# Pi-Star-Lab/RESCO

Hardware: AMD Instinct MI355X
Metric: env-steps/sec (higher is better)
Workload: dtype f32; 1 GPU; ingolstadt21 x 4096 lock-step envs per GPU (BASELINE config 3), fixed demand from the map's rou.xml, on-device seeded random policy, Krauss sigma 0.5 + speedFactor dev 0.1; tls_expiry=1, map=ingolstadt21, envs_per_gpu=4096, pipes=2, ticks_per_env_step=10, block_threads=512, lds_bytes_per_env=40896, parallelism=env-batch split x1, no collective on the data path

## Files before the change

### resco_amd/csrc/resco_step.h

```cpp
#pragma once
#include "resco_tables.h"

struct State {
    char *base;
    size_t nc;
    int32_t *trip_log;
    int32_t *env;
    int32_t *tls;
    long long *stats;
    uint16_t *dep_next;
    uint32_t *mail;
    RS_HD float *pos() const { return (float *)base; }
    RS_HD float *speed() const { return RS_G((float *)(base + 4 * nc)); }
    RS_HD float *accel() const { return RS_G((float *)(base + 8 * nc)); }
    RS_HD float *tloss() const { return RS_G((float *)(base + 12 * nc)); }
    RS_HD float *sf() const { return RS_G((float *)(base + 16 * nc)); }
    RS_HD uint32_t *coop(int par) const { return RS_G((uint32_t *)(base + (par ? 43 : 20) * nc)); }
    RS_HD uint32_t *cooplead(int par) const { return RS_G((uint32_t *)(base + (par ? 47 : 24) * nc)); }
    RS_HD uint16_t *lane() const { return RS_G((uint16_t *)(base + 28 * nc)); }
    RS_HD uint16_t *trip() const { return RS_G((uint16_t *)(base + 30 * nc)); }
    RS_HD uint16_t *cursor() const { return RS_G((uint16_t *)(base + 32 * nc)); }
    RS_HD uint16_t *swait() const { return RS_G((uint16_t *)(base + 34 * nc)); }
    RS_HD uint16_t *rwait() const { return RS_G((uint16_t *)(base + 36 * nc)); }
    RS_HD uint16_t *depart() const { return RS_G((uint16_t *)(base + 38 * nc)); }
// ... 423 lines not shown
template <class LT> RS_DEV Found leader_found(const LT &L, const Grid &grid, int cell0, int ncell, float pos, int k, int self, float win) {
    const int c = cell_of(L, pos, ncell);
    const unsigned long long mykey = order_key(pos, k);
    Found f{(int)NIL, ~0ull, 0u, 0u};
    const uint32_t cw = grid.c[cell0 + c];
    int s = ((cw ^ grid.tag) & CELL_TAG) ? (int)NIL : (int)(cw & NIL);
    if (s == self && ((cw >> CELL_CNT_SHIFT) & CELL_CNT_MAX) == 1u) s = NIL;
    while (s != NIL) {
        RS_ASSERT(s != self || order_key(L.node[s].pos, L.node[s].trip) == mykey)
        RS_CHAIN_STEP(f, s, (key > mykey) & (key < f.key))
    }
    if (f.slot == NIL && c + 1 < ncell) {
        const int cc = scan_up(grid, cell0 + c + 1, cell0 + cell_of(L, pos + win, ncell));
        if (cc >= 0) f = chain_rearmost(L, cell_head(grid, cc));
    }
    if (f.slot != NIL && f.pos() - pos > win) f.slot = NIL;
    return f;
}
template <class LT> RS_DEV int leader_within(const LT &L, const Grid &grid, int cell0, int ncell, float pos, int k, int self, float win) {
    return leader_found(L, grid, cell0, ncell, pos, k, self, win).slot;
}
template <class LT> RS_DEV int follower_within(const LT &L, const Grid &grid, int cell0, int ncell, float pos, int k, int self, float win) {
    const int c = cell_of(L, pos, ncell);
    const unsigned long long mykey = order_key(pos, k);
    Found f{(int)NIL, 0ull, 0u, 0u};
    for (int s = cell_head(grid, cell0 + c); s != NIL;) {
        RS_ASSERT(s != self || order_key(L.node[s].pos, L.node[s].trip) == mykey)
        RS_CHAIN_STEP(f, s, (key < mykey) & (key > f.key))
    }
    if (f.slot == NIL && c > 0) {
        const float lo = pos - win;
        const int cc = scan_down(grid, cell0 + (lo > 0.0f ? cell_of(L, lo, ncell) : 0), cell0 + c - 1);
        if (cc >= 0) f = chain_frontmost(L, cell_head(grid, cc));
    }
    if (f.slot != NIL && pos - f.pos() > win) f.slot = NIL;
    (void)self;
    return f.slot;
}
template <class LT> RS_DEV int at_or_behind_within(const LT &L, const Grid &grid, int cell0, int ncell, float back, float win) {
    if (back < 0.0f) return NIL;
    const int c = cell_of(L, back, ncell);
    Found f{(int)NIL, 0ull, 0u, 0u};
    for (int s = cell_head(grid, cell0 + c); s != NIL;) RS_CHAIN_STEP(f, s, !(nd_.pos > back) & (key > f.key))
    if (f.slot == NIL && c > 0) {
        const float lo = back - win;
        const int cc = scan_down(grid, cell0 + (lo > 0.0f ? cell_of(L, lo, ncell) : 0), cell0 + c - 1);
        if (cc >= 0) f = chain_frontmost(L, cell_head(grid, cc));
    }
    if (f.slot != NIL && back - f.pos() > win) f.slot = NIL;
    return f.slot;
}

template <class LT> RS_DEV int tls_state(const KTab &T, const LT &L, int tls, int pos) {
    if (tls == 0xFF) return TLS_G;
    return L.tstate[tls * T.tls_maxl + pos];
}
RS_DEV uint16_t cache_link(const KTab &T, const LaneRec &LR, int lane, int rq, int trip) {
    if (LR.link_cnt == 0) return NLINK_NONE;
    if (LR.flags & LF_INTERNAL) { const int l = LR.link_start; return (uint16_t)(l | (T.links()[l].arr_idx >= 0 ? NLINK_ARR : 0)); }
    return T.next_link()[((size_t)rq * T.kmax + (lane - (int)LR.edge_lane0)) * 2 + (trip & 1)];
}
template <class LT> RS_DEV bool foe_blocked(const KTab &T, const LT &L, const Grid &grid, const LinkRec &K) {
    for (int i = K.foe_start; i < K.foe_start + K.foe_cnt; ++i) {
        const FoeRec F = rec_load16(T.foes(), i);
        if (F.tls != 0xFF && tls_state(T, L, F.tls, F.tls_pos) == TLS_R) continue;
        if (F.arr_idx >= 0 && L.arr[F.arr_idx] < RM_FOE_GAP_Q) return true;
        if (F.via1_cell0 != 0xFFFF && cells_have_mover(grid, F.via1_cell0, F.via1_nc)) return true;
        if (F.via2_cell0 != 0xFFFF && cells_have_mover(grid, F.via2_cell0, F.via2_nc)) return true;
    }
    return false;
}
template <class LT> RS_DEV void tls_refresh(const KTab &T, const LT &L, const KParams &P, int s, int ph) {
    const int w = T.tls_maxl >> 2;
    const uint32_t *src = (const uint32_t *)((P.fixed_program ? T.cold.fix8 + T.cold.fix_state_off[s] : T.cold.tls8 + T.cold.tls_state_off[s]) + ph * T.tls_maxl);
    uint32_t *dst = (uint32_t *)((uint8_t *)L.tstate + s * T.tls_maxl);
    uint32_t v[8];
#pragma unroll
    for (int i = 0; i < 8; ++i) v[i] = src[i < w ? i : 0];
#pragma unroll
    for (int i = 0; i < 8; ++i) if (i < w) dst[i] = v[i];
#pragma unroll 1
    for (int i = 8; i < w; ++i) dst[i] = src[i];
}
template <class LT> RS_DEV void set_phase(const KTab &T, const LT &L, const KParams &P, int s, int ph) {
    if (ph < 0 || ph >= T.cold.tls_nphase[s]) return;
    L.phase[s] = ph;
    L.left[s] = P.tls_expiry ? T.cold.tls_dur[T.cold.tls_dur_off[s] + ph] : RM_TLS_HOLD_TICKS;
    tls_refresh(T, L, P, s, ph);
}
template <class LT> RS_DEV void tls_begin_of_tick(const KTab &T, const LT &L, const KParams &P, int s, int tick) {
    if (P.do_fsm && !P.fixed_program && tick == T.yellow_length) set_phase(T, L, P, s, L.nextp[s]);
    int left = L.left[s];
    if (left == 0) {
        const int32_t *dur = P.fixed_program ? T.cold.fix_dur + T.cold.fix_dur_off[s] : T.cold.tls_dur + T.cold.tls_dur_off[s];
        const int Pn = P.fixed_program ? T.cold.fix_nphase[s] : T.cold.tls_nphase[s];
        const int ph = (L.phase[s] + 1) % Pn;
        left = dur[ph];
        L.phase[s] = ph;
        tls_refresh(T, L, P, s, ph);
    }
    L.left[s] = left - 1;
}
struct ContRow { float c[4]; const float *cn; };
RS_DEV ContRow cont_row(const KTab &T, int rq) {
    ContRow R;
    R.cn = T.route_cont() + (size_t)rq * T.kmax;
    for (int j = 0; j < 4; ++j) R.c[j] = j < T.kmax ? R.cn[j] : 0.0f;
    return R;
}
RS_DEV float cont_of(const ContRow &R, int j) {
    return j == 0 ? R.c[0] : (j == 1 ? R.c[1] : (j == 2 ? R.c[2] : (j == 3 ? R.c[3] : R.cn[j])));
}
#define OCC_NONE (Grid{(uint16_t *)0, 0u})
#define OCC_FULL (Grid{(uint16_t *)1, 0u})
RS_DEV bool cont_notbest(float c) { return rs_float_as_int(c) < 0; }
RS_DEV float cont_len(float c) { return rs_int_as_float(rs_float_as_int(c) & 0x7FFFFFFF); }
RS_DEV int strategic_dir(const ContRow &R, int kk, int n, float x, float v, int extra, float &rem, const Grid &grid, int cell0, int nc, float occ_unit) {
    const float mine = cont_of(R, kk);
    rem = cont_len(mine) - x;
#ifdef RS_EMU_CHECK_MAIL
    { float best = 0.0f; for (int j = 0; j < n; ++j) { const float c = cont_len(cont_of(R, j)); if (c > best) best = c; }
      for (int j = 0; j < n; ++j) RS_ASSERT(cont_notbest(cont_of(R, j)) == !(cont_len(cont_of(R, j)) >= best - RM_CONT_EPS)) }
#endif
    if (!cont_notbest(mine)) return 0;
    int dl = 1000, dr = 1000;
    for (int j = kk + 1; j < n; ++j) if (!cont_notbest(cont_of(R, j))) { dl = j - kk; break; }
    for (int j = kk - 1; j >= 0; --j) if (!cont_notbest(cont_of(R, j))) { dr = kk - j; break; }
    const int dir = (dr <= dl) ? -1 : +1;
    if (grid.c == (uint16_t *)1) return dir;
    const int off = (dr <= dl ? dr : dl) + extra;
    const float la = (v > RM_LOOK_MIN_SPEED ? v : RM_LOOK_MIN_SPEED) * RM_LOOK_TIME + RM_LOOK_BASE;
    int cnt = 0;
    if (grid.c != (uint16_t *)0) cnt = cells_count(grid, cell0 + ((dr <= dl) ? -dr : dl) * nc, nc);
    if (rem - (float)cnt * occ_unit >= la * (float)off) return 0;
    return dir;
}
RS_DEV uint32_t link_reg_word(const KTab &T, int nlk) { return ((const uint32_t *)&T.links()[nlk & 0x7FFF])[2]; }
template <class LT> RS_DEV void register_approach_w(const KTab &T, const LT &L, uint32_t kw, float v, float pos, float lane_len, int vt) {
    const int st = tls_state(T, L, (int)((kw >> 16) & 0xFFu), (int)(kw >> 24));
    if (st == TLS_R) return;
    const float dist = lane_len - pos;
    if (st == TLS_Y && dist >= d_brake_gap(v, L.vtp[vt * VT_COLS + VT_DECEL])) return;
    const float ta = RS_DIV(dist, v > 1.0f ? v : 1.0f);
    const int q = ta * 10.0f >= 65000.0f ? 65000 : (int)(ta * 10.0f);
    rs_atomic_min(&L.arr[(int16_t)(kw & 0xFFFFu)], q);
}
template <class LT> RS_DEV void register_approach(const KTab &T, const LT &L, int nlk, float v, float pos, float lane_len, int vt) {
    if (!(nlk & NLINK_ARR)) return;
    if (v <= RM_HALT_SPEED) return;
    register_approach_w(T, L, link_reg_word(T, nlk), v, pos, lane_len, vt);
}
template <class LT> RS_DEV void follow_neighbour(const KTab &T, const LT &L, uint32_t key, bool clamp_gap, const LaneRec &LR, int lane, float x, float v,
                             float b, float tau, float mingap, float &vsafe) {
    const int X = (int)(key & 0xFFFFu), kx = (int)(key >> 16);
    if ((int)L.node[X].trip != kx) return;
    const int lx = L.aux[X].lane;
    if (lx == (int)LANE_NONE || (LR.flags & LF_INTERNAL)) return;
    const int l0 = LR.edge_lane0, n = LR.flags >> 2;
    if (lx < l0 || lx >= l0 + n) return;
    const float *vo = L.vtp + L.node[X].vt * VT_COLS;
    const float px = L.node[X].pos, backx = px - vo[VT_LENGTH];
    if (clamp_gap ? !(px >= x) : !(backx >= x)) return;
    float g = backx - x - mingap;
    if (clamp_gap && g < 0.0f) g = 0.0f;
    float vs = d_follow_speed(g, L.node[X].speed, b, vo[VT_DECEL], tau);
    float vc = v - b; if (vc < 0.0f) vc = 0.0f;
    if (vs < vc) vs = vc;
    if (vs < vsafe) vsafe = vs;
    (void)lane;
}

template <class LT> RS_DEV void mail_flag_set(const LT &L, int s, int par) { rs_atomic_or((uint32_t *)((Node *)L.node + s) + 3, SFQ_MAIL(par) << 16); }
template <class LT> RS_DEV void mail_flag_clear(const LT &L, int s, int par) { rs_atomic_and((uint32_t *)((Node *)L.node + s) + 3, ~(SFQ_MAIL(par) << 16)); }
template <class LT, class LP> RS_DEV void list_push(const LT &L, const LP &list, int counter, int s);
template <class LT> RS_DEV void flag_mover(const LT &L, int s, int t, int lct = 0) {
    uint32_t *w = (uint32_t *)((Node *)L.node + s) + 3;
    const uint32_t bit = (uint32_t)fl_mh(t) << 8;
    if (!(rs_atomic_fetch_or(w, bit | ((uint32_t)lct << 8)) & bit)) list_push(L, L.ls_mh, SC_NMH + (t & 1), s);
}
template <class LT, class LP> RS_DEV void list_push(const LT &L, const LP &list, int counter, int s) {
    const int i = rs_wave_ticket(&L.sc[counter]);
    if (i < (int)L.lcap) list[i] = (uint16_t)s;
}
RS_DEV float plan_vfree(const float *vt, float v, float lane_vmax, float sf) {
// ... 348 lines not shown
            }
            if (safe) {
                if (dir == dir_allowed) code = dir > 0 ? LCT_LEFT : LCT_RIGHT;
            } else if (want == 2) {
                if (lead_t != NIL) { G.cooplead(t & 1)[eo + s] = ((uint32_t)L.node[lead_t].trip << 16) | (uint32_t)lead_t; mail_flag_set(L, s, t & 1); }
                const int R = at_or_behind_within(L, grid, tcell0, nc, x - vt[VT_LENGTH], RM_COOP_RANGE);
                if (R != NIL) { rs_atomic_min(&G.coop(t & 1)[eo + R], ((uint32_t)k << 16) | (uint32_t)s); mail_flag_set(L, R, t & 1); }
            }
        }
    }
    if (sdir != 0 && (t % RM_SWAP_EVERY) == 0 && v <= RM_HALT_SPEED && rem <= RM_URGENT_DIST &&
        my_wait >= RM_SWAP_WAIT) {
        const int b = overlapping(L, grid, (int)LR.cell0 + sdir * nc, nc, x, k, s, vt[VT_LENGTH]);
        if (b != NIL) {
            const Node nb = L.node[b];
            float rem_b;
            if (nb.speed <= RM_HALT_SPEED && (int)L.aux[b].swait >= RM_SWAP_WAIT &&
                strategic_dir(cont_row(T, L.aux[b].rq), kk + sdir, n, nb.pos, nb.speed, 0, rem_b, grid, (int)LR.cell0 + sdir * nc, nc, T.occ_unit) == -sdir && rem_b <= RM_URGENT_DIST &&
                overlapping(L, grid, LR.cell0, nc, nb.pos, nb.trip, b, L.vtp[nb.vt * VT_COLS + VT_LENGTH]) == s)
                code |= sdir > 0 ? LCT_SWAP_LEFT : LCT_SWAP_RIGHT;
        }
    }
        return code;
}

template <class LT> RS_DEV bool phase_insert_decide(const KTab &T, const LT &L, const Grid &grid, int t, int d) {
    if ((int)L.dep_t[d] > t) return false;
    const int k = L.dep[d];
    const DepInfo LR = rec_load8(T.cold.dep_info, d);
    const float *vt = L.vtp + T.trip_vtype()[k] * VT_COLS;
    const float mypos = vt[VT_LENGTH] < LR.len ? vt[VT_LENGTH] : LR.len;
    const int nc = (int)(LR.len * L.cell_inv) + 1;
    const int c1 = LR.cell0 + cell_of(L, mypos + vt[VT_MINGAP] + T.maxlen, nc);
    for (int c = scan_up(grid, LR.cell0, c1); c >= 0; c = (c < c1 ? scan_up(grid, c + 1, c1) : -1))
        for (int o = cell_head(grid, c); o != NIL;) { RS_CHAIN_GUARD
            const Node od = L.node[o];
            const float back = (od.pos + L.vnx[o]) - L.vtp[od.vt * VT_COLS + VT_LENGTH];
            if (back - mypos - vt[VT_MINGAP] < 0.0f) return false;
            o = od.nxt;
        }
    return true;
}

template <class LT> RS_DEV int nth_free_slot(const LT &L, int C, int r) {
#pragma unroll 1
    for (int w = 0; w < (C + 31) / 32; ++w) {
        uint32_t fr = ~L.alive0[w];
        if (w == (C - 1) / 32 && (C & 31)) fr &= (1u << (C & 31)) - 1u;
        const int c = rs_popc(fr);
        if (r >= c) { r -= c; continue; }
#pragma unroll 1
        for (int j = 0; j < r; ++j) fr &= fr - 1u;
        return w * 32 + rs_ffs(fr) - 1;
    }
    return -1;
}

template <class LT> RS_DEV void lc_decide_and_flag(const KTab &T, const LT &L, const Grid &grid, const State &G, size_t eo, int t, int s) {
    const Aux ax = L.aux[s];
    if (ax.lane == LANE_NONE) return;
    const int code = phase_lc_decide(T, L, grid, G, eo, t, s, ax, L.node[s]);
    if (code) flag_mover(L, s, t, code);
}
struct ExecInline {};

template <int CAP, class Exec, class LT>
RS_DEV void rs_step_body_on(Exec &ex, const LT &L, const KTab &T, const State &G, const Out &O, const KParams &P,
                            const int32_t *actions, int env) {
    const int B = ex.B;
    const int C = CAP ? CAP : T.capacity, S = T.n_signals, NO = T.n_obs;
    const int genv = P.env_base + env;
    const size_t eo = (size_t)env * C;
    const int n_ticks = P.n_ticks;

    uint16_t *const grid0 = L.grid;

    ex.phase(0, [&](int tid) {
        if (tid < SC_STATS + ST_N) L.sc[tid] = tid < 4 ? G.env[env * 4 + tid] : 0;
        for (int i = tid; i < T.n_vtypes * VT_COLS; i += B) L.vtp[i] = T.cold.vtype_params[i];
        for (int i = tid; i < (int)(L.gstride >> 1); i += B) ((uint32_t *)grid0)[i] = 0x07FF07FFu;
        for (int i = tid; i < T.n_arr; i += B) L.arr[i] = ARR_NONE;
        for (int i = tid; i < (C + 31) / 32; i += B) { L.alive[i] = 0u; L.mailw[i] = 0u; }
        for (int i = tid; i < (T.n_dep + 31) / 32; i += B) L.insm[i] = 0u;
        for (int i = tid; i < T.n_dep; i += B) {
            const int k = G.dep_next[(size_t)env * T.n_dep + i];
            L.dep[i] = (uint16_t)k;
            L.dep_t[i] = k == (int)TRIP_NONE ? (uint16_t)0xFFFF : (uint16_t)T.cold.trip_depart[k];
        }
        for (int i = tid; i < S; i += B) {
            const int ph = G.tls[(env * S + i) * TLS_W + 0];
            L.phase[i] = ph;
            L.left[i] = G.tls[(env * S + i) * TLS_W + 1];
            L.nextp[i] = G.tls[(env * S + i) * TLS_W + 2];
            L.sig_arr[i] = 0; L.sig_dep[i] = G.tls[(env * S + i) * TLS_W + 3];
            tls_refresh(T, L, P, i, ph);
        }
    });
    ex.phase(1, [&](int tid) {
        const int hw0 = L.sc[SC_HW];
        for (int s = tid; s < C; s += B) {
            uint16_t ln = LANE_NONE, tr = TRIP_NONE;
            if (s < hw0) { ln = G.lane()[eo + s]; tr = G.trip()[eo + s]; }
            Aux ax; ax.lane = ln; ax.rq = 0; ax.nlink = NLINK_NONE; ax.swait = 0;
            if (ln == LANE_NONE) { L.aux[s] = ax; L.node[s].trip = TRIP_NONE; continue; }
            const float sp = G.speed()[eo + s], x = G.pos()[eo + s];
            const int rq = (int)T.routes()[T.trip_route()[tr]].start + (int)G.cursor()[eo + s];
            const LaneRec LR0 = rec_load16(T.lanes(), ln);
            ax.rq = (uint16_t)rq;
            ax.nlink = cache_link(T, LR0, ln, rq, tr);
            ax.swait = G.swait()[eo + s];
            L.aux[s] = ax;
            Node nn; nn.pos = x; nn.speed = sp; nn.trip = tr; nn.vt = T.trip_vtype()[tr];
            nn.fl = 0; nn.sfq = (uint16_t)speed_factor_q(P, genv, tr, L.vtp + nn.vt * VT_COLS);
            if ((G.mail[(size_t)env * ((C + 31) / 32) + (s >> 5)] >> (s & 31)) & 1u) nn.sfq |= (uint16_t)SFQ_MAIL((L.sc[SC_T] + 1) & 1);
            nn.nxt = grid_push(Grid{grid0, 0u}, LR0.cell0 + cell_of(L, x, lane_cells(L, LR0)), s, sp > RM_HALT_SPEED);
            if (n_ticks > 0) nn.fl = (uint8_t)classify(T, L, s, L.vtp + nn.vt * VT_COLS, sp, x, LR0, ln, rq, T.notbest()[rq], tr, sf_of(nn.sfq), L.sc[SC_T]);
            L.node[s] = nn;
            rs_atomic_or(&L.alive[s >> 5], 1u << (s & 31));
        }
        for (int s = B - 1 - tid; s < S; s += B) {
            if (P.do_fsm && !P.fixed_program) {
                const int a = actions[env * S + s], cur = L.phase[s], Gn = T.cold.tls_ngreen[s];
                if (a < 0 || a >= T.cold.tls_nphase[s]) L.nextp[s] = cur;
                else {
                    L.nextp[s] = a;
                    if (cur != a && cur < Gn && a < Gn) {
                        const int y = T.cold.tls_yellow[T.cold.tls_yel_off[s] + cur * Gn + a];
                        if (y >= 0) set_phase(T, L, P, s, y);
                    }
                }
            }
            if (n_ticks > 0) tls_begin_of_tick(T, L, P, s, 0);
        }
    });
    if (n_ticks > 0) ex.phase(2, [&](int tid) {
        const int hw = L.sc[SC_HW];
        for (int s = tid; s < hw; s += B) {
            const Aux ax = L.aux[s];
            if (ax.lane == LANE_NONE) continue;
            const Node me = L.node[s];
            register_approach(T, L, ax.nlink, me.speed, me.pos, T.lanes()[ax.lane].len, me.vt);
        }
    });

    int cur = 0;
    for (int tick = 0; tick < n_ticks; ++tick) {
        const int t = L.sc[SC_T], hw = L.sc[cur ? SC_HWNEW : SC_HW];
        const Grid gold{grid0, cur ? CELL_TAG : 0u}, gnew{grid0, cur ? 0u : CELL_TAG};
        const bool more = tick + 1 < n_ticks;
        const int lcap = (int)L.lcap;
        const int nwv = B >> 6;
        ex.phase(4, [&](int tid) {
            const int wv = ex.wave_of(tid), ln = tid & 63;
            const int nh = L.sc[SC_NH], nlc = L.sc[SC_NLC];
            const unsigned long long r0 = ex.role_begin();
            int role = 0;
            if (nh > lcap || nlc > lcap) {
                for (int pass = 0; pass < 2; ++pass)
                    for (int w = tid; w < hw; w += B) {
                        if (pass && !(L.node[w].fl & FL_LC)) continue;
                        if (pass) lc_decide_and_flag(T, L, gold, G, eo, t, w);
                        else phase_plan<true>(T, L, gold, G, eo, P, genv, t, w);
                    }
            } else {
                const int hch = (nh + RS_H_CHUNK - 1) / RS_H_CHUNK, lch = (nlc + RS_LIST_CHUNK - 1) / RS_LIST_CHUNK;
                const int total = hch + lch + ((hw + 63) >> 6);
                for (int it = 0;; ++it) {
                    const int c = ex.next_chunk(&L.sc[SC_CHUNK_P], wv, it, nwv);
                    if (c >= total) break;
                    if (c < hch) {
                        role = 1;
                        const int w = c * RS_H_CHUNK + ln;
                        if (ln < RS_H_CHUNK && w < nh) phase_plan<true>(T, L, gold, G, eo, P, genv, t, L.ls_h[w]);
                    } else if (c < hch + lch) {
                        role = 2;
                        const int w = (c - hch) * RS_LIST_CHUNK + ln;
                        if (ln < RS_LIST_CHUNK && w < nlc) lc_decide_and_flag(T, L, gold, G, eo, t, L.ls_lc[w]);
                    } else {
                        const int w = (c - hch - lch) * 64 + ln;
                        if (w < hw && !(L.node[w].fl & FL_H)) phase_plan<false>(T, L, gold, G, eo, P, genv, t, w);
                    }
                }
            }
            ex.role_end(role == 1 ? 7 : (role == 2 ? 8 : 9), r0);
            for (int i = tid; i < (T.n_dep + 31) / 32; i += B) L.insm[i] = 0u;
        });
        ex.phase(5, [&](int tid) {
            for (int i = tid; i < T.n_arr; i += B) L.arr[i] = ARR_NONE;
            for (int i = tid; i < (C + 31) / 32; i += B) L.alive0[i] = L.alive[i];
            int Bs = B;
            RS_OPAQUE_S(Bs)
            for (int i = tid; i < (int)(L.gstride >> 2); i += Bs) {
                unsigned long long *q = (unsigned long long *)grid0 + i;
                const unsigned long long w = *q;
                const unsigned long long st = ((w ^ grid_tag4(gold)) >> 15) & 0x0001000100010001ull;
                if (st) { const unsigned long long m = st * 0xFFFFull; *q = (w & ~m) | ((0x07FF07FF07FF07FFull | grid_tag4(gold)) & m); }
            }
            for (int d = B - 1 - tid; d < T.n_dep; d += B)
                if (phase_insert_decide(T, L, gold, t, d)) rs_atomic_or(&L.insm[d >> 5], 1u << (d & 31));
            if (more)
                for (int sg = B - 1 - tid; sg < S; sg += B) tls_begin_of_tick(T, L, P, sg, tick + 1);
            if (tid == 0) {
                L.sc[SC_T] = t + 1; L.sc[SC_STATS + ST_TICKS] += 1;
                L.sc[cur ? SC_HW : SC_HWNEW] = 0;
                L.sc[SC_ROOM] = C - L.sc[SC_NACT];
                L.sc[SC_NH] = 0; L.sc[SC_NLC] = 0;
                L.sc[SC_NMH + ((t + 1) & 1)] = 0;
                L.sc[SC_CHUNK_P] = 0; L.sc[SC_CHUNK_M] = 0;
            }
        });
        ex.phase(6, [&](int tid) {
            int active = 0, halted = 0, top = 0;
            const int wv = ex.wave_of(tid), ln = tid & 63;
            const int nmh = L.sc[SC_NMH + (t & 1)];
            int ich = 0;
// ... 35 lines not shown
                        L.aux[s] = na;
                        G.sf()[eo + s] = sfn; G.tloss()[eo + s] = 0.0f; G.cooplead(0)[eo + s] = COOP_NONE; G.cooplead(1)[eo + s] = COOP_NONE; G.coop(0)[eo + s] = COOP_NONE; G.coop(1)[eo + s] = COOP_NONE;
                        G.rwait()[eo + s] = 0; G.owner()[eo + s] = OWNER_NONE; G.depart()[eo + s] = (uint16_t)(t + 1); G.accel()[eo + s] = 0.0f; G.wtot()[eo + s] = 0;
                        {
                            const int k2 = T.cold.trip_next[k];
                            L.dep[d] = (uint16_t)k2;
                            L.dep_t[d] = k2 == (int)TRIP_NONE ? (uint16_t)0xFFFF : (uint16_t)T.cold.trip_depart[k2];
                        }
                        rs_atomic_or(&L.alive[s >> 5], 1u << (s & 31));
                        rs_atomic_add(&L.sc[SC_NACT], 1);
                        rs_atomic_add(&L.sc[SC_NINS], 1);
                        rs_atomic_add(&L.sc[SC_STATS + ST_INSERTED], 1);
                        rs_atomic_add(&L.sc[SC_STATS + ST_DEPDELAY], t - T.cold.trip_depart[k]);
                        if (s + 1 > top) top = s + 1;
                    }
                } else {
                    const int w = (c - mch - ich) * 64 + ln;
                    if (w < hw && (L.alive0[w >> 5] & (1u << (w & 31)))) {
                        if (all) phase_move<true>(T, L, gnew, G, P, env, eo, t, !more, more, w, active, halted, top);
                        else if (!(L.node[w].fl & fl_mh(t))) phase_move<false>(T, L, gnew, G, P, env, eo, t, !more, more, w, active, halted, top);
                    }
                }
            }
            ex.role_end(list ? 10 : 3, r0);
            rs_wave_add(&L.sc[SC_STATS + ST_ACTIVE_TICKS], active);
            rs_wave_add(&L.sc[SC_STATS + ST_WAITING], halted);
            rs_wave_max(&L.sc[cur ? SC_HW : SC_HWNEW], top);
            ex.role_end(15, r0);
        });
        cur ^= 1;
    }
    const int hw_end = L.sc[cur ? SC_HWNEW : SC_HW];

    const bool obs = P.do_observe != 0;
    if (obs) ex.phase(11, [&](int tid) {
        for (int i = tid; i < NO; i += B) { L.agg_q[i] = 0; L.agg_a[i] = 0; L.agg_w[i] = 0; L.agg_m[i] = 0; L.agg_s[i] = 0; L.agg_n[i] = 0; }
    });
    ex.phase(12, [&](int tid) {
        const int hw0 = G.env[env * 4 + 2];
        const int top = hw_end > hw0 ? hw_end : hw0;
        int hi = 0;
        for (int s = tid; s < top; s += B) {
            const int lane = L.aux[s].lane;
            G.lane()[eo + s] = (uint16_t)lane; G.trip()[eo + s] = L.node[s].trip;
            if (lane == (int)LANE_NONE) continue;
            hi = s + 1;
            if (L.node[s].sfq & SFQ_MAIL((L.sc[SC_T] + 1) & 1)) rs_atomic_or(&L.mailw[s >> 5], 1u << (s & 31));
            const int rq = L.aux[s].rq;
            G.pos()[eo + s] = L.node[s].pos; G.speed()[eo + s] = L.node[s].speed; G.swait()[eo + s] = L.aux[s].swait;
            G.cursor()[eo + s] = (uint16_t)(rq - (int)T.routes()[T.trip_route()[L.node[s].trip]].start);
            if (!obs) continue;
            const int prev_owner = G.owner()[eo + s];
            const LaneRec LR = T.lanes()[lane];
            const int oi = T.cold.lane_obs[lane];
            bool detect = false;
            if (oi >= 0) {
                const float d = (LR.len - L.node[s].pos) + T.rsteps()[rq].tlsdist;
                detect = d <= P.max_distance;
            }
            if (!detect) {
                if (prev_owner != (int)OWNER_NONE) rs_atomic_add(&L.sig_dep[prev_owner], 1);
                G.owner()[eo + s] = OWNER_NONE; G.rwait()[eo + s] = 0;
                continue;
            }
            const int sig = T.cold.obs_sig[oi];
            int rw = G.rwait()[eo + s];
            if (prev_owner != sig) {
                rw = 0;
                rs_atomic_add(&L.sig_arr[sig], 1);
                rs_atomic_add(&L.agg_n[oi], 1);
                if (prev_owner != (int)OWNER_NONE) rs_atomic_add(&L.sig_dep[prev_owner], 1);
            }
            if (rw > 0) { rw += T.step_length; if (rw > 65535) rw = 65535; }
            else { const int sw = L.aux[s].swait; if (sw > 0) rw = sw; }
            G.rwait()[eo + s] = (uint16_t)rw;
            G.owner()[eo + s] = (uint8_t)sig;
            if (rw > 0) { rs_atomic_add(&L.agg_q[oi], 1); rs_atomic_add(&L.agg_w[oi], rw); rs_atomic_max(&L.agg_m[oi], rw); }
            else rs_atomic_add(&L.agg_a[oi], 1);
            rs_atomic_add((int32_t *)&L.agg_s[oi], (int32_t)(uint32_t)(L.node[s].speed * 65536.0f + 0.5f));
        }
        if (hi) rs_atomic_max(&L.sc[SC_HWOUT], hi);
    });
    ex.phase(13, [&](int tid) {
        const uint32_t om = obs ? P.out_mask : 0u;
        if (om & (OUT_LANE_AGG | OUT_DRQ_NORM)) for (int i = tid; i < NO * 5; i += B) {
            const int oi = i / 5, c = i - oi * 5;
            const int sg = T.cold.obs_sig[oi];
            const float sp = (float)L.agg_s[oi] * (1.0f / 65536.0f);
            float raw, nrm;
            if (c == 0) { raw = (float)L.agg_q[oi]; nrm = (oi - T.cold.sig_obs_start[sg]) == L.phase[sg] ? 1.0f : 0.0f; }
            else if (c == 1) { raw = (float)L.agg_a[oi]; nrm = raw / 28.0f; }
            else if (c == 2) { raw = (float)L.agg_w[oi]; nrm = raw / 28.0f; }
            else if (c == 3) { raw = (float)L.agg_m[oi]; nrm = (float)L.agg_q[oi] / 28.0f; }
            else { raw = sp; nrm = sp / 20.0f / 28.0f; }
            if (om & OUT_LANE_AGG) O.lane_agg()[(size_t)env * NO * 5 + i] = raw;
            if (om & OUT_DRQ_NORM) O.drq_norm()[(size_t)env * NO * 5 + i] = nrm;
        }
        if (om & OUT_LANE_ARR) for (int i = tid; i < NO; i += B) O.lane_arr()[(size_t)env * NO + i] = L.agg_n[i];
        if (om & OUT_DRQ_F16) for (int i = tid; i < S * T.lmax * 5; i += B) {
            const int sg = i / (T.lmax * 5), r = i - sg * T.lmax * 5;
            const int l = r / 5, c = r - l * 5;
            const int o0 = T.cold.sig_obs_start[sg];
            float nrm = 0.0f;
            if (l < T.cold.sig_obs_start[sg + 1] - o0) {
                const int oi = o0 + l;
                if (c == 0) nrm = l == L.phase[sg] ? 1.0f : 0.0f;
                else if (c == 1) nrm = (float)L.agg_a[oi] / 28.0f;
                else if (c == 2) nrm = (float)L.agg_w[oi] / 28.0f;
                else if (c == 3) nrm = (float)L.agg_q[oi] / 28.0f;
                else nrm = (float)L.agg_s[oi] * (1.0f / 65536.0f) / 20.0f / 28.0f;
            }
            O.drq_f16()[(size_t)env * S * T.lmax * 5 + i] = rs_f2h(nrm);
        }
        if (om & (OUT_MPLIGHT | OUT_WAVE | OUT_MPLIGHT_FULL)) for (int i = tid; i < S * 12; i += B) {
            const int sg = i / 12, m = i - sg * 12;
            int q = 0, wv = 0, tw = 0, ap = 0;
            float last_speed = 0.0f;
            for (int j = T.cold.mv_in_start[i]; j < T.cold.mv_in_start[i + 1]; ++j) {
                const int oi = T.cold.mv_in_idx[j];
                q += L.agg_q[oi]; wv += L.agg_q[oi] + L.agg_a[oi]; tw += L.agg_w[oi]; ap += L.agg_a[oi];
                last_speed = (float)L.agg_s[oi] * (1.0f / 65536.0f);
            }
            for (int j = T.cold.mv_out_start[i]; j < T.cold.mv_out_start[i + 1]; ++j) q -= L.agg_q[T.cold.mv_out_idx[j]];
            const size_t so = (size_t)env * S + sg;
            if (om & OUT_MPLIGHT) O.mplight()[so * 13 + 1 + m] = q;
            if (om & OUT_WAVE) O.wave()[so * 12 + m] = wv;
            if (om & OUT_MPLIGHT_FULL) {
                float *mf = O.mplight_full() + so * 49 + 1 + m * 4;
                mf[0] = (float)q; mf[1] = (float)tw / 28.0f; mf[2] = last_speed; mf[3] = (float)ap / 28.0f;
            }
        }
        for (int sg = tid; sg < S; sg += B) {
            const int ph = L.phase[sg];
            if (obs) {
                const int o0 = T.cold.sig_obs_start[sg], o1 = T.cold.sig_obs_start[sg + 1];
                int tw = 0, tq = 0, mq = 0;
                for (int oi = o0; oi < o1; ++oi) { tw += L.agg_w[oi]; const int qq = L.agg_q[oi]; tq += qq; if (qq > mq) mq = qq; }
                const size_t so = (size_t)env * S + sg;
                O.phase()[so] = ph; O.queue_sum()[so] = tq; O.queue_max()[so] = mq;
                O.wait()[so] = -(float)tw;
                const float wn = -(float)tw / 224.0f;
                O.wait_norm()[so] = wn < -4.0f ? -4.0f : (wn > 4.0f ? 4.0f : wn);
                int pr = tq;
                for (int i = T.cold.pr_out_start[sg]; i < T.cold.pr_out_start[sg + 1]; ++i) pr -= L.agg_q[T.cold.pr_out_idx[i]];
                O.pressure()[so] = -pr;
                if (om & OUT_MPLIGHT) O.mplight()[so * 13] = ph;
                if (om & OUT_MPLIGHT_FULL) O.mplight_full()[so * 49] = (float)ph;
                O.arrivals()[so] = L.sig_arr[sg]; O.departures()[so] = L.sig_dep[sg];
            }
            G.tls[(env * S + sg) * TLS_W + 0] = ph;
            G.tls[(env * S + sg) * TLS_W + 1] = L.left[sg];
            G.tls[(env * S + sg) * TLS_W + 2] = L.nextp[sg];
            G.tls[(env * S + sg) * TLS_W + 3] = obs ? 0 : L.sig_dep[sg];
        }
        for (int i = tid; i < T.n_dep; i += B) G.dep_next[(size_t)env * T.n_dep + i] = L.dep[i];
        for (int i = tid; i < (C + 31) / 32; i += B) G.mail[(size_t)env * ((C + 31) / 32) + i] = L.mailw[i];
    });
    ex.phase(14, [&](int tid) {
        if (tid == 0) {
            G.env[env * 4 + 0] = L.sc[SC_T]; G.env[env * 4 + 1] = L.sc[SC_NINS]; G.env[env * 4 + 3] = L.sc[SC_NACT];
            G.env[env * 4 + 2] = L.sc[SC_HWOUT];
        }
        if (tid < ST_N) {
            long long *st = G.stats + (size_t)env * ST_N;
            if (tid == ST_ACTIVE) st[tid] = L.sc[SC_NACT];
            else if (tid == ST_PENDING) {
                const int t = L.sc[SC_T];
                const int hz = t - 1 <= T.horizon ? t - 1 : T.horizon;
                st[tid] = (t >= 1 ? T.cold.trips_cum[hz] : 0) - L.sc[SC_NINS];
            } else st[tid] += L.sc[SC_STATS + tid];
        }
    });
}

template <int CAP, class Exec>
RS_DEV void rs_step_body(Exec &ex, const Lds &L, const KTab &T, const State &G, const Out &O, const KParams &P,
                         const int32_t *actions, int env) {
    if constexpr (CAP != 0) {
        const LdsFix<CAP> Lf(L);
        rs_step_body_on<CAP>(ex, Lf, T, G, O, P, actions, env);
    } else rs_step_body_on<CAP>(ex, L, T, G, O, P, actions, env);
}
```

### resco_amd/csrc/resco_tables.h

```cpp
#pragma once
#include <stdint.h>
#include <string.h>
#include <string>
#include <vector>

#include "resco_model.h"
#include "resco_sim.h"

enum { VT_LENGTH, VT_MINGAP, VT_ACCEL, VT_DECEL, VT_TAU, VT_SIGMA, VT_MAXSPEED, VT_SF_MEAN, VT_SF_DEV, VT_EMERGENCY, VT_COLS };
enum { TLS_R = 0, TLS_Y = 1, TLS_g = 2, TLS_G = 3 };
enum { ST_INSERTED, ST_ARRIVED, ST_DURATION, ST_DEPDELAY, ST_WAITING, ST_TLOSS, ST_ACTIVE, ST_PENDING, ST_ACTIVE_TICKS, ST_TICKS, ST_CAP_BLOCKED, ST_INVARIANT, ST_N };

#define LANE_NONE 0xFFFFu
#define OWNER_NONE 0xFFu
#define NIL 0x7FF
#define CELL_CNT_SHIFT 11
#define CELL_CNT_MAX 7u
#define CELL_MOVER 0x4000u
#define CELL_TAG 0x8000u
#define ARR_NONE 65535
#define COOP_NONE 0xFFFFFFFFu
#define TRIP_NONE 0xFFFFu

#ifdef CELL_LEN
// ... 32 lines not shown
};
struct __attribute__((aligned(16))) RouteRec {
    uint32_t start;
    uint16_t depart_lane;
    int16_t dep_idx;
    uint16_t depart_cell0;
    uint16_t pad;
    float depart_len;
};
#define LF_INTERNAL 1u
#define KF_MINOR 1u
#define KF_CONT 2u
#define NLINK_NONE 0x7FFF
#define NLINK_ARR 0x8000

struct __attribute__((aligned(8))) DepInfo { float len; uint16_t cell0, lane; };
struct KCold {
    const int32_t *trip_depart;
    const uint16_t *trip_next;
    const uint16_t *dep_lane;
    const struct DepInfo *dep_info;
    const uint16_t *dep_first;
    const float *vtype_params;
    const uint8_t *tls8, *fix8;
    const int32_t *tls_nphase, *tls_ngreen, *tls_nlinks, *tls_state_off, *tls_dur_off, *tls_yel_off, *tls_dur, *tls_yellow, *tls_init_phase;
    const int32_t *fix_nphase, *fix_state_off, *fix_dur_off, *fix_dur, *fix_init_phase, *fix_init_left;
    const int16_t *lane_obs;
    const int32_t *obs_sig, *sig_obs_start, *mv_in_start, *mv_in_idx, *mv_out_start, *mv_out_idx, *pr_out_start, *pr_out_idx;
    const int32_t *trips_cum;
};
#ifndef RS_G
#define RS_G(p) (p)
#endif
#ifndef RS_MEM
#define RS_MEM inline
#endif
#ifndef RS_KEEP4
#define RS_KEEP4(a, b, c, d)
#endif
#ifndef RS_KEEP2
#define RS_KEEP2(a, b)
#endif
static_assert(sizeof(LaneRec) == 16 && alignof(LaneRec) == 16, "LaneRec: one 16-byte load");
static_assert(sizeof(FoeRec) == 16 && alignof(FoeRec) == 16, "FoeRec: one 16-byte load");
static_assert(sizeof(RouteRec) == 16 && alignof(RouteRec) == 16, "RouteRec: one 16-byte load");
static_assert(sizeof(LinkRec) == 32 && alignof(LinkRec) == 16, "LinkRec: two 16-byte loads");
static_assert(sizeof(RStep) == 8 && alignof(RStep) == 8, "RStep: one 8-byte load");
static_assert(sizeof(DepInfo) == 8 && alignof(DepInfo) == 8, "DepInfo: one 8-byte load");
#ifdef RS_FIELD_LOADS
#define rec_load16(tab, i) ((tab)[i])
#define rec_load8(tab, i) ((tab)[i])
#define link_load(tab, i) ((tab)[i])
#else
struct alignas(16) RecRaw16 { uint32_t a, b, c, d; };
template <class R, class I> RS_MEM R rec_load16(const R *tab, I i) {
    static_assert(sizeof(R) == 16 && alignof(R) == 16, "rec_load16: a 16-byte record");
    RecRaw16 r;
    __builtin_memcpy(&r, &tab[i], 16);
    RS_KEEP4(r.a, r.b, r.c, r.d)
    R out;
    __builtin_memcpy(&out, &r, 16);
    return out;
}
template <class R, class I> RS_MEM R rec_load8(const R *tab, I i) {
    static_assert(sizeof(R) == 8 && alignof(R) == 8, "rec_load8: an 8-byte record");
    struct alignas(8) Raw { uint32_t a, b; } r;
    __builtin_memcpy(&r, &tab[i], 8);
    RS_KEEP2(r.a, r.b)
    R out;
    __builtin_memcpy(&out, &r, 8);
    return out;
}
template <class I> RS_MEM LinkRec link_load(const LinkRec *tab, I i) {
    RecRaw16 r[2];
    __builtin_memcpy(r, &tab[i], 32);
    RS_KEEP4(r[0].a, r[0].b, r[0].c, r[0].d)
    RS_KEEP4(r[1].a, r[1].b, r[1].c, r[1].d)
    LinkRec out;
    __builtin_memcpy(&out, r, 32);
    return out;
}
#endif

struct KTab {
    const LaneRec *lanes_;
    const LinkRec *links_;
    const FoeRec *foes_;
    const RStep *rsteps_;
    const float *route_cont_;
    const uint16_t *next_link_;
    const uint16_t *notbest_;
    const RouteRec *routes_;
    const uint16_t *trip_route_;
    const uint8_t *trip_vtype_;
    KCold cold;
    float maxlen;
    float occ_unit;
    int32_t n_trips, tls_maxl, kmax;
    int32_t n_lanes, n_cells, n_signals, n_obs, n_vtypes, horizon, capacity, step_length, yellow_length, lmax, n_arr, n_dep;
    RS_MEM const LaneRec *lanes() const { return RS_G(lanes_); }
    RS_MEM const LinkRec *links() const { return RS_G(links_); }
    RS_MEM const FoeRec *foes() const { return RS_G(foes_); }
    RS_MEM const RStep *rsteps() const { return RS_G(rsteps_); }
    RS_MEM const float *route_cont() const { return RS_G(route_cont_); }
    RS_MEM const uint16_t *next_link() const { return RS_G(next_link_); }
    RS_MEM const uint16_t *notbest() const { return RS_G(notbest_); }
    RS_MEM const RouteRec *routes() const { return RS_G(routes_); }
    RS_MEM const uint16_t *trip_route() const { return RS_G(trip_route_); }
    RS_MEM const uint8_t *trip_vtype() const { return RS_G(trip_vtype_); }
};

struct KParams {
    uint32_t seed;
    int32_t env_base;
    float max_distance, sigma;
    int32_t speed_dev, fixed_program;
    int32_t tls_expiry;
    int32_t n_ticks;
    int32_t do_fsm;
    int32_t do_observe;
    uint32_t out_mask;
    int32_t n_envs;
    unsigned long long *prof;
};

#define OUT_LANE_AGG 1u
#define OUT_DRQ_NORM 2u
#define OUT_DRQ_F16 4u
#define OUT_LANE_ARR 8u
#define OUT_MPLIGHT 16u
#define OUT_WAVE 32u
#define OUT_MPLIGHT_FULL 64u
#define OUT_VEH_ACCEL 128u
#define OUT_ALL 255u
#define TLS_W 4

struct PackedTables {
    std::vector<LaneRec> lanes;
    std::vector<LinkRec> links;
    std::vector<FoeRec> foes;
    std::vector<RStep> rsteps;
    std::vector<RouteRec> routes;
    std::vector<uint16_t> next_link, trip_route, trip_next, dep_lane, dep_first, notbest;
    std::vector<uint8_t> trip_vtype, tls8, fix8;
    std::vector<DepInfo> dep_info;
    std::vector<int32_t> tls_off_p, fix_off_p;
    std::vector<int16_t> lane_obs16;
    std::vector<int32_t> obs_sig;
    std::vector<float> route_cont;
    int n_cells = 0, n_arr = 1, n_dep = 1, kmax = 1, lmax = 1, tls_maxl = 1;
    float maxlen = 0.0f, occ_unit = 0.0f;
    float cell_len = 30.0f, cell_inv = 1.0f / 30.0f;
    std::string err;

    static void choose(const rs_scenario *sc, int q, int ln, int out[2]) {
        out[0] = out[1] = -1;
        const int ne = sc->route_edge[q + 1];
        const float *cn = sc->route_cont + (size_t)(q + 1) * sc->kmax;
        float bc = -1.0f;
        for (int l = sc->lane_link_start[ln]; l < sc->lane_link_start[ln] + sc->lane_link_cnt[ln]; ++l) {
            if (sc->link_to_edge[l] != ne) continue;
            const float c = cn[sc->link_dest_lane[l] - sc->edge_lane0[ne]];
            if (c > bc) bc = c;
        }
        if (bc < RM_MIN_LC_LEN) return;
        int n = 0;
// ... 188 lines not shown
```

Baseline: 3.986 million env-steps/s.

## Batch vehicle state loads, defer TLS refresh, and spread writeback roles across wavefronts

The vehicle load phase now handles two slots per thread and issues all global loads (lane, trip, cursor, speed, position, mail, route, lane record, next-link) up front in dependent batches, so memory latency overlaps instead of being serialized per vehicle. The TLS phase-state copy is deferred so it runs at most once per signal per step rather than on both the yellow transition and the tick start. The final writeback phase merges phases 13 and 14, removing one barrier, and assigns each output group to a different starting wavefront through rotated indices so the groups run on different waves in parallel. Risks are higher register pressure from the doubled per-thread state and more complex index mapping.

```diff
diff --git a/resco_amd/csrc/resco_step.h b/resco_amd/csrc/resco_step.h
--- a/resco_amd/csrc/resco_step.h
+++ b/resco_amd/csrc/resco_step.h
@@ -529,14 +529,16 @@
 #pragma unroll 1
     for (int i = 8; i < w; ++i) dst[i] = src[i];
 }
-template <class LT> RS_DEV void set_phase(const KTab &T, const LT &L, const KParams &P, int s, int ph) {
-    if (ph < 0 || ph >= T.cold.tls_nphase[s]) return;
+template <class LT> RS_DEV int set_phase(const KTab &T, const LT &L, const KParams &P, int s, int ph, bool refresh = true) {
+    if (ph < 0 || ph >= T.cold.tls_nphase[s]) return -1;
     L.phase[s] = ph;
     L.left[s] = P.tls_expiry ? T.cold.tls_dur[T.cold.tls_dur_off[s] + ph] : RM_TLS_HOLD_TICKS;
-    tls_refresh(T, L, P, s, ph);
-}
-template <class LT> RS_DEV void tls_begin_of_tick(const KTab &T, const LT &L, const KParams &P, int s, int tick) {
-    if (P.do_fsm && !P.fixed_program && tick == T.yellow_length) set_phase(T, L, P, s, L.nextp[s]);
+    if (refresh) tls_refresh(T, L, P, s, ph);
+    return ph;
+}
+template <class LT> RS_DEV int tls_begin_of_tick(const KTab &T, const LT &L, const KParams &P, int s, int tick, bool refresh = true) {
+    int now = -1;
+    if (P.do_fsm && !P.fixed_program && tick == T.yellow_length) now = set_phase(T, L, P, s, L.nextp[s], refresh);
     int left = L.left[s];
     if (left == 0) {
         const int32_t *dur = P.fixed_program ? T.cold.fix_dur + T.cold.fix_dur_off[s] : T.cold.tls_dur + T.cold.tls_dur_off[s];
@@ -544,9 +546,11 @@
         const int ph = (L.phase[s] + 1) % Pn;
         left = dur[ph];
         L.phase[s] = ph;
-        tls_refresh(T, L, P, s, ph);
+        if (refresh) tls_refresh(T, L, P, s, ph);
+        now = ph;
     }
     L.left[s] = left - 1;
+    return now;
 }
 struct ContRow { float c[4]; const float *cn; };
 RS_DEV ContRow cont_row(const KTab &T, int rq) {
@@ -1061,12 +1065,12 @@
         for (int i = tid; i < T.n_arr; i += B) L.arr[i] = ARR_NONE;
         for (int i = tid; i < (C + 31) / 32; i += B) { L.alive[i] = 0u; L.mailw[i] = 0u; }
         for (int i = tid; i < (T.n_dep + 31) / 32; i += B) L.insm[i] = 0u;
-        for (int i = tid; i < T.n_dep; i += B) {
+        for (int i = rs_role_index(B, B - 1 - tid, B > 64 ? 64 : 0); i < T.n_dep; i += B) {
             const int k = G.dep_next[(size_t)env * T.n_dep + i];
             L.dep[i] = (uint16_t)k;
             L.dep_t[i] = k == (int)TRIP_NONE ? (uint16_t)0xFFFF : (uint16_t)T.cold.trip_depart[k];
         }
-        for (int i = tid; i < S; i += B) {
+        for (int i = B - 1 - tid; i < S; i += B) {
             const int ph = G.tls[(env * S + i) * TLS_W + 0];
             L.phase[i] = ph;
             L.left[i] = G.tls[(env * S + i) * TLS_W + 1];
@@ -1077,39 +1081,82 @@
     });
     ex.phase(1, [&](int tid) {
         const int hw0 = L.sc[SC_HW];
-        for (int s = tid; s < C; s += B) {
-            uint16_t ln = LANE_NONE, tr = TRIP_NONE;
-            if (s < hw0) { ln = G.lane()[eo + s]; tr = G.trip()[eo + s]; }
-            Aux ax; ax.lane = ln; ax.rq = 0; ax.nlink = NLINK_NONE; ax.swait = 0;
-            if (ln == LANE_NONE) { L.aux[s] = ax; L.node[s].trip = TRIP_NONE; continue; }
-            const float sp = G.speed()[eo + s], x = G.pos()[eo + s];
-            const int rq = (int)T.routes()[T.trip_route()[tr]].start + (int)G.cursor()[eo + s];
-            const LaneRec LR0 = rec_load16(T.lanes(), ln);
-            ax.rq = (uint16_t)rq;
-            ax.nlink = cache_link(T, LR0, ln, rq, tr);
-            ax.swait = G.swait()[eo + s];
-            L.aux[s] = ax;
-            Node nn; nn.pos = x; nn.speed = sp; nn.trip = tr; nn.vt = T.trip_vtype()[tr];
-            nn.fl = 0; nn.sfq = (uint16_t)speed_factor_q(P, genv, tr, L.vtp + nn.vt * VT_COLS);
-            if ((G.mail[(size_t)env * ((C + 31) / 32) + (s >> 5)] >> (s & 31)) & 1u) nn.sfq |= (uint16_t)SFQ_MAIL((L.sc[SC_T] + 1) & 1);
-            nn.nxt = grid_push(Grid{grid0, 0u}, LR0.cell0 + cell_of(L, x, lane_cells(L, LR0)), s, sp > RM_HALT_SPEED);
-            if (n_ticks > 0) nn.fl = (uint8_t)classify(T, L, s, L.vtp + nn.vt * VT_COLS, sp, x, LR0, ln, rq, T.notbest()[rq], tr, sf_of(nn.sfq), L.sc[SC_T]);
-            L.node[s] = nn;
-            rs_atomic_or(&L.alive[s >> 5], 1u << (s & 31));
+        const size_t mo = (size_t)env * ((C + 31) / 32);
+        for (int sa = tid; sa < C; sa += 2 * B) {
+            const bool two = sa + B < C;
+            const int sl[2] = {sa, two ? sa + B : sa};
+            uint32_t ln[2], tr[2], cu[2], sw[2], ml[2];
+            float sp[2], x[2];
+#pragma unroll
+            for (int j = 0; j < 2; ++j) {
+                const int s = sl[j];
+                ln[j] = G.lane()[eo + s]; tr[j] = G.trip()[eo + s]; cu[j] = G.cursor()[eo + s]; sw[j] = G.swait()[eo + s];
+                sp[j] = G.speed()[eo + s]; x[j] = G.pos()[eo + s]; ml[j] = G.mail[mo + (s >> 5)];
+            }
+            RS_KEEP4(ln[0], tr[0], cu[0], sw[0]) RS_KEEP4(ln[1], tr[1], cu[1], sw[1]) RS_KEEP4(sp[0], x[0], sp[1], x[1]) RS_KEEP2(ml[0], ml[1])
+            bool live[2];
+            uint32_t rt[2], vt[2];
+            LaneRec LR[2];
+#pragma unroll
+            for (int j = 0; j < 2; ++j) {
+                if (sl[j] >= hw0) { ln[j] = LANE_NONE; tr[j] = TRIP_NONE; }
+                live[j] = ln[j] != LANE_NONE;
+                rt[j] = T.trip_route()[live[j] ? tr[j] : 0u]; vt[j] = T.trip_vtype()[live[j] ? tr[j] : 0u];
+                LR[j] = rec_load16(T.lanes(), live[j] ? ln[j] : 0u);
+            }
+            RS_KEEP4(rt[0], vt[0], rt[1], vt[1])
+            uint32_t rq[2];
+#pragma unroll
+            for (int j = 0; j < 2; ++j) rq[j] = T.routes()[live[j] ? rt[j] : 0u].start;
+            RS_KEEP2(rq[0], rq[1])
+            uint32_t nb[2], nl[2];
+            int32_t la[2];
+#pragma unroll
+            for (int j = 0; j < 2; ++j) {
+                rq[j] = live[j] ? rq[j] + cu[j] : 0u;
+                const bool internal = (LR[j].flags & LF_INTERNAL) != 0;
+                const bool normal = live[j] && LR[j].link_cnt != 0 && !internal;
+                nb[j] = T.notbest()[rq[j]];
+                nl[j] = T.next_link()[normal ? (rq[j] * (uint32_t)T.kmax + (ln[j] - (uint32_t)LR[j].edge_lane0)) * 2u + (tr[j] & 1u) : 0u];
+                la[j] = T.links()[live[j] && LR[j].link_cnt != 0 && internal ? LR[j].link_start : 0].arr_idx;
+            }
+            RS_KEEP4(nb[0], nl[0], nb[1], nl[1]) RS_KEEP2(la[0], la[1])
+#pragma unroll
+            for (int j = 0; j < 2; ++j) {
+                const int s = sl[j];
+                if (j == 1 && !two) break;
+                Aux ax; ax.lane = (uint16_t)ln[j]; ax.rq = 0; ax.nlink = NLINK_NONE; ax.swait = 0;
+                if (!live[j]) { L.aux[s] = ax; L.node[s].trip = TRIP_NONE; continue; }
+                const LaneRec &LR0 = LR[j];
+                ax.rq = (uint16_t)rq[j];
+                if (LR0.link_cnt != 0) ax.nlink = (LR0.flags & LF_INTERNAL) ? (uint16_t)(LR0.link_start | (la[j] >= 0 ? NLINK_ARR : 0)) : (uint16_t)nl[j];
+                ax.swait = (uint16_t)sw[j];
+                L.aux[s] = ax;
+                Node nn; nn.pos = x[j]; nn.speed = sp[j]; nn.trip = (uint16_t)tr[j]; nn.vt = (uint8_t)vt[j];
+                nn.fl = 0; nn.sfq = (uint16_t)speed_factor_q(P, genv, (int)tr[j], L.vtp + nn.vt * VT_COLS);
+                if ((ml[j] >> (s & 31)) & 1u) nn.sfq |= (uint16_t)SFQ_MAIL((L.sc[SC_T] + 1) & 1);
+                nn.nxt = grid_push(Grid{grid0, 0u}, LR0.cell0 + cell_of(L, x[j], lane_cells(L, LR0)), s, sp[j] > RM_HALT_SPEED);
+                if (n_ticks > 0) nn.fl = (uint8_t)classify(T, L, s, L.vtp + nn.vt * VT_COLS, sp[j], x[j], LR0, (int)ln[j], (int)rq[j], nb[j], (int)tr[j], sf_of(nn.sfq), L.sc[SC_T]);
+                L.node[s] = nn;
+                rs_atomic_or(&L.alive[s >> 5], 1u << (s & 31));
+            }
         }
         for (int s = B - 1 - tid; s < S; s += B) {
+            const int ph0 = L.phase[s];
+            int ph1 = ph0;
             if (P.do_fsm && !P.fixed_program) {
-                const int a = actions[env * S + s], cur = L.phase[s], Gn = T.cold.tls_ngreen[s];
+                const int a = actions[env * S + s], cur = ph0, Gn = T.cold.tls_ngreen[s];
                 if (a < 0 || a >= T.cold.tls_nphase[s]) L.nextp[s] = cur;
                 else {
                     L.nextp[s] = a;
                     if (cur != a && cur < Gn && a < Gn) {
                         const int y = T.cold.tls_yellow[T.cold.tls_yel_off[s] + cur * Gn + a];
-                        if (y >= 0) set_phase(T, L, P, s, y);
+                        if (y >= 0) { const int r = set_phase(T, L, P, s, y, false); if (r >= 0) ph1 = r; }
                     }
                 }
             }
-            if (n_ticks > 0) tls_begin_of_tick(T, L, P, s, 0);
+            if (n_ticks > 0) { const int r = tls_begin_of_tick(T, L, P, s, 0, false); if (r >= 0) ph1 = r; }
+            if (ph1 != ph0) tls_refresh(T, L, P, s, ph1);
         }
     });
     if (n_ticks > 0) ex.phase(2, [&](int tid) {
@@ -1311,8 +1358,9 @@
         if (hi) rs_atomic_max(&L.sc[SC_HWOUT], hi);
     });
     ex.phase(13, [&](int tid) {
+        enum { NR = 8, R_ROWS = 0, R_MAIL = 1, R_TLS = 2, R_DEP = 3, R_ENV = 4, R_SIG = 5, R_MV = 6, R_ARR = 7 };
         const uint32_t om = obs ? P.out_mask : 0u;
-        if (om & (OUT_LANE_AGG | OUT_DRQ_NORM)) for (int i = tid; i < NO * 5; i += B) {
+        if (om & (OUT_LANE_AGG | OUT_DRQ_NORM)) for (int i = rs_role_index(B, tid, rs_role_first(B, R_ROWS, NR)); i < NO * 5; i += B) {
             const int oi = i / 5, c = i - oi * 5;
             const int sg = T.cold.obs_sig[oi];
             const float sp = (float)L.agg_s[oi] * (1.0f / 65536.0f);
@@ -1325,8 +1373,8 @@
             if (om & OUT_LANE_AGG) O.lane_agg()[(size_t)env * NO * 5 + i] = raw;
             if (om & OUT_DRQ_NORM) O.drq_norm()[(size_t)env * NO * 5 + i] = nrm;
         }
-        if (om & OUT_LANE_ARR) for (int i = tid; i < NO; i += B) O.lane_arr()[(size_t)env * NO + i] = L.agg_n[i];
-        if (om & OUT_DRQ_F16) for (int i = tid; i < S * T.lmax * 5; i += B) {
+        if (om & OUT_LANE_ARR) for (int i = rs_role_index(B, tid, rs_role_first(B, R_ARR, NR)); i < NO; i += B) O.lane_arr()[(size_t)env * NO + i] = L.agg_n[i];
+        if (om & OUT_DRQ_F16) for (int i = rs_role_index(B, tid, rs_role_first(B, R_ROWS, NR)); i < S * T.lmax * 5; i += B) {
             const int sg = i / (T.lmax * 5), r = i - sg * T.lmax * 5;
             const int l = r / 5, c = r - l * 5;
             const int o0 = T.cold.sig_obs_start[sg];
@@ -1341,7 +1389,7 @@
             }
             O.drq_f16()[(size_t)env * S * T.lmax * 5 + i] = rs_f2h(nrm);
         }
-        if (om & (OUT_MPLIGHT | OUT_WAVE | OUT_MPLIGHT_FULL)) for (int i = tid; i < S * 12; i += B) {
+        if (om & (OUT_MPLIGHT | OUT_WAVE | OUT_MPLIGHT_FULL)) for (int i = rs_role_index(B, tid, rs_role_first(B, R_MV, NR)); i < S * 12; i += B) {
             const int sg = i / 12, m = i - sg * 12;
             int q = 0, wv = 0, tw = 0, ap = 0;
             float last_speed = 0.0f;
@@ -1359,45 +1407,46 @@
                 mf[0] = (float)q; mf[1] = (float)tw / 28.0f; mf[2] = last_speed; mf[3] = (float)ap / 28.0f;
             }
         }
-        for (int sg = tid; sg < S; sg += B) {
+        if (obs) for (int sg = rs_role_index(B, tid, rs_role_first(B, R_SIG, NR)); sg < S; sg += B) {
             const int ph = L.phase[sg];
-            if (obs) {
-                const int o0 = T.cold.sig_obs_start[sg], o1 = T.cold.sig_obs_start[sg + 1];
-                int tw = 0, tq = 0, mq = 0;
-                for (int oi = o0; oi < o1; ++oi) { tw += L.agg_w[oi]; const int qq = L.agg_q[oi]; tq += qq; if (qq > mq) mq = qq; }
-                const size_t so = (size_t)env * S + sg;
-                O.phase()[so] = ph; O.queue_sum()[so] = tq; O.queue_max()[so] = mq;
-                O.wait()[so] = -(float)tw;
-                const float wn = -(float)tw / 224.0f;
-                O.wait_norm()[so] = wn < -4.0f ? -4.0f : (wn > 4.0f ? 4.0f : wn);
-                int pr = tq;
-                for (int i = T.cold.pr_out_start[sg]; i < T.cold.pr_out_start[sg + 1]; ++i) pr -= L.agg_q[T.cold.pr_out_idx[i]];
-                O.pressure()[so] = -pr;
-                if (om & OUT_MPLIGHT) O.mplight()[so * 13] = ph;
-                if (om & OUT_MPLIGHT_FULL) O.mplight_full()[so * 49] = (float)ph;
-                O.arrivals()[so] = L.sig_arr[sg]; O.departures()[so] = L.sig_dep[sg];
-            }
-            G.tls[(env * S + sg) * TLS_W + 0] = ph;
+            const int o0 = T.cold.sig_obs_start[sg], o1 = T.cold.sig_obs_start[sg + 1];
+            int tw = 0, tq = 0, mq = 0;
+            for (int oi = o0; oi < o1; ++oi) { tw += L.agg_w[oi]; const int qq = L.agg_q[oi]; tq += qq; if (qq > mq) mq = qq; }
+            const size_t so = (size_t)env * S + sg;
+            O.phase()[so] = ph; O.queue_sum()[so] = tq; O.queue_max()[so] = mq;
+            O.wait()[so] = -(float)tw;
+            const float wn = -(float)tw / 224.0f;
+            O.wait_norm()[so] = wn < -4.0f ? -4.0f : (wn > 4.0f ? 4.0f : wn);
+            int pr = tq;
+            for (int i = T.cold.pr_out_start[sg]; i < T.cold.pr_out_start[sg + 1]; ++i) pr -= L.agg_q[T.cold.pr_out_idx[i]];
+            O.pressure()[so] = -pr;
+            if (om & OUT_MPLIGHT) O.mplight()[so * 13] = ph;
+            if (om & OUT_MPLIGHT_FULL) O.mplight_full()[so * 49] = (float)ph;
+            O.arrivals()[so] = L.sig_arr[sg]; O.departures()[so] = L.sig_dep[sg];
+        }
+        for (int sg = rs_role_index(B, tid, rs_role_first(B, R_TLS, NR)); sg < S; sg += B) {
+            G.tls[(env * S + sg) * TLS_W + 0] = L.phase[sg];
             G.tls[(env * S + sg) * TLS_W + 1] = L.left[sg];
             G.tls[(env * S + sg) * TLS_W + 2] = L.nextp[sg];
             G.tls[(env * S + sg) * TLS_W + 3] = obs ? 0 : L.sig_dep[sg];
         }
-        for (int i = tid; i < T.n_dep; i += B) G.dep_next[(size_t)env * T.n_dep + i] = L.dep[i];
-        for (int i = tid; i < (C + 31) / 32; i += B) G.mail[(size_t)env * ((C + 31) / 32) + i] = L.mailw[i];
-    });
-    ex.phase(14, [&](int tid) {
-        if (tid == 0) {
-            G.env[env * 4 + 0] = L.sc[SC_T]; G.env[env * 4 + 1] = L.sc[SC_NINS]; G.env[env * 4 + 3] = L.sc[SC_NACT];
-            G.env[env * 4 + 2] = L.sc[SC_HWOUT];
-        }
-        if (tid < ST_N) {
-            long long *st = G.stats + (size_t)env * ST_N;
-            if (tid == ST_ACTIVE) st[tid] = L.sc[SC_NACT];
-            else if (tid == ST_PENDING) {
-                const int t = L.sc[SC_T];
-                const int hz = t - 1 <= T.horizon ? t - 1 : T.horizon;
-                st[tid] = (t >= 1 ? T.cold.trips_cum[hz] : 0) - L.sc[SC_NINS];
-            } else st[tid] += L.sc[SC_STATS + tid];
+        for (int i = rs_role_index(B, tid, rs_role_first(B, R_DEP, NR)); i < T.n_dep; i += B) G.dep_next[(size_t)env * T.n_dep + i] = L.dep[i];
+        for (int i = rs_role_index(B, tid, rs_role_first(B, R_MAIL, NR)); i < (C + 31) / 32; i += B) G.mail[(size_t)env * ((C + 31) / 32) + i] = L.mailw[i];
+        {
+            const int i = rs_role_index(B, tid, rs_role_first(B, R_ENV, NR));
+            if (i == 0) {
+                G.env[env * 4 + 0] = L.sc[SC_T]; G.env[env * 4 + 1] = L.sc[SC_NINS]; G.env[env * 4 + 3] = L.sc[SC_NACT];
+                G.env[env * 4 + 2] = L.sc[SC_HWOUT];
+            }
+            if (i < ST_N) {
+                long long *st = G.stats + (size_t)env * ST_N;
+                if (i == ST_ACTIVE) st[i] = L.sc[SC_NACT];
+                else if (i == ST_PENDING) {
+                    const int t = L.sc[SC_T];
+                    const int hz = t - 1 <= T.horizon ? t - 1 : T.horizon;
+                    st[i] = (t >= 1 ? T.cold.trips_cum[hz] : 0) - L.sc[SC_NINS];
+                } else st[i] += L.sc[SC_STATS + i];
+            }
         }
     });
 }
diff --git a/resco_amd/csrc/resco_tables.h b/resco_amd/csrc/resco_tables.h
--- a/resco_amd/csrc/resco_tables.h
+++ b/resco_amd/csrc/resco_tables.h
@@ -138,6 +138,9 @@
 }
 #endif
 
+RS_MEM int rs_role_first(int B, int r, int n) { return ((r * (B >> 6)) / n) << 6; }
+RS_MEM int rs_role_index(int B, int tid, int first) { const int i = tid - first; return i < 0 ? i + B : i; }
+
 struct KTab {
     const LaneRec *lanes_;
     const LinkRec *links_;
```

Result: no change. 4.006 million env-steps/s (median of 6 runs) (+0.5%).
